# unmeshvrije/scikit-kge

Hardware: AMD Instinct MI355X
Metric: triples/sec (score+grad+update), WN18 TransE d=200, 1/2/4/8 MI355X (higher is better)
Workload: dtype f32; 1 GPU; TransE-L1 d=200 PairwiseStochasticTrainer+AdaGrad, WN18 shape, nb=100 (B=1414), margin 2.0, lr 0.1, device RandomModeSampler(1,[0,1]); step = 1 epoch; global_batch=1414, parallelism=1gpu

## Files before the change

### scikit-kge_amd/csrc/skge_pipe_plan.h

```cpp
#pragma once
#include <stddef.h>
#include <stdint.h>

#include <algorithm>
#include <vector>

#include "../../include/skge_hip.h"
#include "skge_epoch_batches.h"

namespace skge {

constexpr int HOT_REPS = 4, HOT_MIN = 4, HOT_REL = 8, HOT_MAX = 256;

constexpr int SLOT_BUF = 1 << 30;

constexpr int PIPE_WG_GRP = 192;
#ifndef SKGE_PIPE_WG
#define SKGE_PIPE_WG 256
#endif

constexpr int HPIPE_OCC = 2;

struct PipeEnv {
  int fused = -1;
  int rreps = 0;
  bool hole_fft = false;
  bool hole_hot = true;
  size_t lds_fft_wave = 0, lds_fft_wg = 0, lds_direct_wg = 0;
  int shard_words = 0;
};

struct PipeLaunch {
  long long start;
  int count, prev_slots, pprev_slots, nwork, nA, grid;
};

struct PipeBytes {
  size_t ent_rows = 0;
  size_t ent_sum = 0;
  size_t ent_word = 0;
  size_t ent_meta = 0;
  size_t slots = 0;
  size_t rel_rows = 0;
  size_t rel_acc = 0;
  size_t rec = 0, rec_n1 = 0, err = 0, key_copy = 0, stats = 0, viol = 0;
  size_t hot_sum = 0, hot_cnt = 0, hot_val = 0, hot_row = 0;
};

struct PipePlan {
  bool hole = false;
  bool dp = false;
  bool e8 = false;
  bool w32 = false;
  bool grouped = false;
  bool fused = false;
  bool fft = false;
  bool pair = false;
  bool hot = false;
  bool ent_ada = false, rel_ada = false;
  int kq = 1;
  int reps = 1, rw = 0;
  bool rfold = false;
  size_t lds = 0;
  int wpb = 0;
  int hw = 0;
  int N = 0, M = 0, d = 0, nb1 = 0;
  long long T = 0;
  int64_t bs = 0;
  EpochBatches batches;
  std::vector<PipeLaunch> launch;
  PipeBytes bytes;

  int threads() const { return pair ? 128 : (grouped ? PIPE_WG_GRP : SKGE_PIPE_WG); }
  int nlaunch() const { return nb1 + 3; }
  int kernel() const { return hole ? 2 : (fused ? 1 : 0); }

  int score_groups(int n) const {
    if (n <= 0) return 0;
    return pair ? std::max(1, std::min(n, 2 * 16384))
                : std::max(1, std::min((n + wpb - 1) / wpb, 16384));
  }
// ... 26 lines not shown
    const int cprev = b >= 1 ? (int)batches[b - 1].second : 0;
    a.prev_slots = 4 * cprev;
    if (p.fused) {
      const int cpp = b >= 2 ? (int)batches[b - 2].second : 0;
      a.pprev_slots = 4 * cpp;
      a.nwork = a.count + std::max(cprev, cpp);
      a.nA = 0;
      a.grid = std::max(1, (p.M + a.nwork + WPB - 1) / WPB);
      p.launch.push_back(a);
      continue;
    }
    const int a_items = p.M + nhot +
                        (p.hole ? 4 * cprev
                         : p.grouped ? (4 * cprev + 63) / 64 : 4 * cprev);
    auto nBwaves = [&](long long cnt) { return p.pair ? 2 * cnt : (cnt + WPB - 1) / WPB * WPB; };
    const int occ = p.pair ? std::max(4, HPIPE_OCC) : p.fft ? 4 : HPIPE_OCC;
    int a_cap = p.hole && b < nb1 ? std::max(1, (occ * 4 * 256 - (int)nBwaves(batches[b].second)) / WPB - 8) : 16384;
    if (p.hole && b < nb1 && (long long)nBwaves(batches[b].second) > occ * 4 * 256)
      a_cap = std::max(a_cap, 256);
    a.nA = std::max(1, std::min((a_items + WPB - 1) / WPB, std::min(a_cap, 16384)));
    a.grid = a.nA + p.score_groups(a.count);
    p.launch.push_back(a);
  }
}

inline PipePlan pipe_plan(const skge_table_t* ent, const skge_table_t* rel, int d, int64_t T,
                          int nbatches, int flags, bool hole, const PipeEnv& env) {
  PipePlan p;
  p.hole = hole;
  p.dp = (flags & SKGE_PIPE_DP) != 0;
  p.batches = epoch_batches(T, nbatches);
  p.nb1 = p.batches.size();
  p.bs = p.batches.bs;
  p.T = T;
  p.d = d;
  const int64_t bs = p.bs, maxb = p.batches.maxb;
  const int nq = d / 4;
  const int N = p.N = ent->rows, M = p.M = rel->rows;
  p.fft = hole && env.hole_fft;
  p.pair = p.fft && d == 200 && 2 * maxb <= 4 * 4 * 256;
  p.e8 = !hole && ent->acc_mode == SKGE_ACC_I8X4;
  p.w32 = rel->acc_mode == SKGE_ACC_I32X2;
  p.kq = (nq + 63) / 64;
  p.grouped = !hole && 4 * bs > 4 * 4096;
  {
    const bool ok = !hole && !p.grouped && nq <= 64 && (long long)N < SLOT_BUF;
    p.fused = ok && !p.dp && (env.fused >= 0 ? env.fused != 0 : nq <= 16);
  }
  p.hot = !p.fused && !p.e8 && !p.dp && (!hole || (p.pair && env.hole_hot));
  p.hw = ((hole ? d / 2 : nq) + 15) / 16 * 16;
  p.ent_ada = ent->opt == SKGE_ADAGRAD && ent->state != nullptr;
  p.rel_ada = rel->opt == SKGE_ADAGRAD;
  p.reps = 1;
  if (hole)
    while (p.reps < 32 && (long long)p.reps * 2048 < bs) p.reps *= 2;
  if (hole && env.rreps) p.reps = std::max(1, env.rreps);
  if (p.grouped) {
    const long long per_row = bs / std::max(1, M);
    while (p.reps < 16 && (long long)p.reps * 256 < per_row) p.reps *= 2;
  }
  p.rfold = p.reps > 1;
  p.rw = hole ? ((d + 2) / 2 + 15) / 16 * 16 : ((p.w32 ? 2 * nq : nq) + 1 + 15) / 16 * 16;
  p.lds = !hole ? 0 : p.pair ? env.lds_fft_wave : p.fft ? env.lds_fft_wg : env.lds_direct_wg;
  p.wpb = p.pair ? 2 : (p.grouped ? PIPE_WG_GRP : SKGE_PIPE_WG) / 64;

  PipeBytes& b = p.bytes;
  b.ent_rows = (size_t)N * d * 4;
  b.ent_sum = (size_t)N * nq * (hole ? 16 : (p.e8 ? 4 : 8));
  b.ent_word = (size_t)N * 4;
  b.ent_meta = (size_t)N * 16;
  b.slots = (size_t)4 * bs * 4;
  b.rel_rows = (size_t)M * d * 4;
// ... 17 lines not shown
```

### scikit-kge_amd/csrc/skge_pipeline.hip

```cpp
#include <algorithm>
#include <cstdlib>
#include <tuple>
#include <type_traits>
#include <vector>

#include "skge_graph_runner.h"
#include "skge_hole.h"
#include "skge_hole_fft.h"
#include "skge_pipe.h"
#include "skge_sampler.h"
#include "skge_transe_l1.h"

namespace skge {

#ifndef SKGE_HPIPE_HOT
#define SKGE_HPIPE_HOT 1
#endif

#ifndef SKGE_PIPE_WAVES_I8
#define SKGE_PIPE_WAVES_I8 7
#endif
#ifndef SKGE_PIPE_WAVES_I16
#define SKGE_PIPE_WAVES_I16 7
#endif
constexpr int pipe_batch_waves(int kq, bool w32, bool e8, bool grp, bool hot, bool dp) {
  return (kq != 1 || w32 || grp || hot || dp) ? 0 : (e8 ? SKGE_PIPE_WAVES_I8 : SKGE_PIPE_WAVES_I16);
}
template <int KQ, bool W32, bool E8, bool GRP = false, bool HOT = false, bool DP = false>
__global__ __launch_bounds__(GRP ? PIPE_WG_GRP : SKGE_PIPE_WG)
__attribute__((amdgpu_waves_per_eu(pipe_batch_waves(KQ, W32, E8, GRP, HOT, DP),
                                   pipe_batch_waves(KQ, W32, E8, GRP, HOT, DP))))
void k_pipe_batch(PipeArgs a) {
  const int wpb = blockDim.x >> 6;
  const int l = lane_id();
  const int d = a.d, nq = d >> 2;
  const int rcw = W32 ? 2 * nq : nq;
  const int g = launch_id(a), gp = g - 1;
  const int cp = a.b & 1, pp = cp ^ 1;
  const int rd = a.b & 1;
  const int rw = a.b < a.nb1 ? rd ^ 1 : 0;
  const int ra_prev = (g - 1) % 3, ra_cur = g % 3, ra_old = (g - 2) % 3;
  const int nB = (int)gridDim.x - a.nA;
  const int blk = (int)blockIdx.x;
  const int blk_a = blk, blk_b = blk - a.nA;
  if (blk < a.nA) {
    const int nR = a.R.rows;
    const int* const ownp = a.E.own[pp];
    const int nH = a.E.nhot, nRH = nR + nH;
    const int total = nRH + (ownp ? (a.prev_slots + 63) / 64 : a.prev_slots);
    const int wa = blk_a * wpb + (threadIdx.x >> 6);
    const unsigned long long ta0 = a.trace ? now_10ns() : 0ull;
    const bool wt = a.b < a.nb1;
    if (a.b == a.nb1 && wa == 0) {
      fold_shards(a.nviol_shards, a.nviol_total);
      advance_key(a);
    }
    for (int w = wa; w < total; w += a.nA * wpb) {
      if (w < nR) {
        rel_publish<KQ, W32>(a, w, rd, rw, ra_prev, ra_old);
      } else if (w < nRH) {
        if (HOT) apply_hot<KQ>(a.E, w - nR, g, d);
      } else if (ownp) {
        const int i = 64 * (w - nRH) + l;
        const int r = i < a.prev_slots ? a.E.touched[pp][i] : -1;
        const bool mine = r >= 0 && ownp[r] == i;
        uint64_t m = __ballot(mine);
        if (GRP) {
          while (m) {
            const int rank = __popcll(m & ((1ull << l) - 1ull));
            const bool take = ((m >> l) & 1ull) && rank < GRP_ROWS;
            const uint64_t tk = __ballot(take);
            const int n = __popcll(tk);
            int src = 0;
            {
              uint64_t t2 = tk;
              for (int j = 0; j < GRP_ROWS && t2; ++j) {
                const int k = __ffsll((unsigned long long)t2) - 1;
                t2 &= t2 - 1;
                if (l == j) src = k;
              }
            }
            const int rl = __builtin_amdgcn_ds_bpermute(src << 2, r);
            claim_and_apply_rows<KQ, E8>(a.E, pp, rl, n, d, gp, wt);
            m &= ~tk;
          }
        } else {
          while (m) {
            const int k = __ffsll((unsigned long long)m) - 1;
            m &= m - 1;
            const int row = __builtin_amdgcn_readlane(r, k);
            claim_and_apply<KQ, E8>(a.E, pp, row, d, gp, wt);
          }
        }
      } else {
        const int row = __builtin_amdgcn_readfirstlane(a.E.touched[pp][w - nRH]);
        if (row >= 0) claim_and_apply<KQ, E8>(a.E, pp, row, d, gp, wt);
      }
    }
    if (a.trace && l == 0) {
      unsigned long long* tr = a.trace + 2 + 6 * (size_t)a.count + 2 * (size_t)wa;
      tr[0] = ta0;
      tr[1] = now_10ns();
    }
    return;
  }
  int* const cnt_cp = opaque_ptr(a.E.cnt[cp]);
  int* const tch_cp = opaque_ptr(a.E.touched[cp]);
  int* const pend_cp = opaque_ptr(a.E.pend[cp]);
  int* const own_cp = a.E.own[cp];
  unsigned long long* const racc0 = opaque_ptr(a.R.acc[ra_cur]);
  const size_t rrep = (size_t)a.R.rows * a.R.rw;
  const int rmask = a.R.reps - 1;
  unsigned long long* const esum = opaque_ptr(a.E.sum[cp]);
  const __amdgpu_buffer_rsrc_t rec_rs = __builtin_amdgcn_make_buffer_rsrc(
      const_cast<int4*>(a.rec + a.start), 0, a.count * 16, 0x00020000);
  const __amdgpu_buffer_rsrc_t rec1_rs = __builtin_amdgcn_make_buffer_rsrc(
      const_cast<int*>(a.rec_n1 + a.start), 0, a.count * 4, 0x00020000);
  int nv = 0;
  const int lo = DP ? a.lo : 0, hi = DP ? a.hi : a.count;
  for (int w = lo + blk_b * wpb + (threadIdx.x >> 6); w < hi; w += nB * wpb) {
    unsigned long long* const racc = racc0 + (size_t)(w & rmask) * rrep;
    unsigned long long tt[4];
    if (a.trace) tt[0] = now_10ns();
    const u32x4 rx = __builtin_amdgcn_raw_buffer_load_b128(rec_rs, w * 16, 0, 0);
    const int r1 = (int)__builtin_amdgcn_raw_buffer_load_b32(rec1_rs, w * 4, 0, 0);
    const int4 r4 = make_int4((int)rx.x, (int)rx.y, (int)rx.z, (int)rx.w);
    __builtin_amdgcn_sched_barrier(0);
    const int s = __builtin_amdgcn_readfirstlane(r4.x);
    const int o = __builtin_amdgcn_readfirstlane(r4.y);
    const int p = __builtin_amdgcn_readfirstlane(r4.z);
    const int neg0 = __builtin_amdgcn_readfirstlane(r4.w);
    const int neg1 = __builtin_amdgcn_readfirstlane(r1);
    const int n0r = neg0 >= 0 ? neg0 : s, n1r = neg1 >= 0 ? neg1 : o;
    float4 es[KQ], eo[KQ], rp[KQ], fs[KQ], fo[KQ], ra[KQ];
    unsigned long long rsv[KQ], rsw[KQ], rcnt;
    rel_row_issue<KQ, W32>(a.R, p, d, rd, ra_prev, rp, ra, rsv, rsw, rcnt);
    __builtin_amdgcn_sched_barrier(0);
    load_row4_buf<KQ>(a.E.P, s, d, es);
    load_row4_buf<KQ>(a.E.P, o, d, eo);
    load_row4_buf<KQ>(a.E.P, n0r, d, fs);
    load_row4_buf<KQ>(a.E.P, n1r, d, fo);
    const int rr = sel4(l & 3, s, o, n0r, n1r);
    const int mark = a.E.pend[pp][rr];
    const int dn = __hip_atomic_load(a.E.done + rr, __ATOMIC_RELAXED, __HIP_MEMORY_SCOPE_AGENT);
    int hx = -1;
    if (HOT) hx = a.E.hot[rr];
    __builtin_amdgcn_sched_barrier(0);
    {
      int c;
      rel_row_finish<KQ, W32>(a.R, d, rsv, rsw, rcnt, rp, ra, c);
    }
    __builtin_amdgcn_sched_barrier(0);
    const uint64_t pend = __ballot(mark == gp) & 0xfull;
    const uint64_t unpub = pend & ~__ballot(dn == gp);
    if (a.trace) tt[1] = now_10ns();
    if (pend) {
#pragma unroll 1
      for (int k = 0; k < 4; ++k) {
        if (!((unpub >> k) & 1ull)) continue;
        ensure_applied<KQ, E8>(a.E, pp, sel4(k, s, o, n0r, n1r), d, gp, a.err);
      }
      if (pend & 1ull) load_row4_sc1<KQ>(a.E.P, s, d, es);
      if (pend & 2ull) load_row4_sc1<KQ>(a.E.P, o, d, eo);
      if (pend & 4ull) load_row4_sc1<KQ>(a.E.P, n0r, d, fs);
      if (pend & 8ull) load_row4_sc1<KQ>(a.E.P, n1r, d, fo);
    }
    if (HOT) {
      const uint64_t hm = __ballot(hx >= 0) & 0xfull;
#pragma unroll 1
      for (int k = 0; k < 4; ++k) {
        if (!((hm >> k) & 1ull)) continue;
        float4 hv[KQ], ha[KQ];
        hot_value<KQ>(a.E, __builtin_amdgcn_readlane(hx, k), g, d, hv, ha);
#pragma unroll
        for (int m = 0; m < KQ; ++m) {
          if (k == 0) es[m] = hv[m];
          if (k == 1) eo[m] = hv[m];
          if (k == 2) fs[m] = hv[m];
          if (k == 3) fo[m] = hv[m];
        }
      }
    }
    if (a.trace) tt[2] = now_10ns();
    float ps, n0, n1;
    float4 gp4[KQ], g0[KQ], g1[KQ];
    int v0, v1;
    l1_scores_signs<KQ>(es, eo, fs, fo, rp, ps, n0, n1, gp4, g0, g1);
    l1_decide(ps, n0, n1, neg0, neg1, a.margin, v0, v1);
    if (a.trace) tt[3] = now_10ns();
    if (DP && a.dprec) {
      uint32_t* out = a.dprec + (size_t)(w - lo) * pipe_dp_record_words(d);
      if (l == 0) out[0] = (uint32_t)(v0 | (v1 << 1));
      if (v0 + v1 > 0) {
#pragma unroll
        for (int m = 0; m < KQ; ++m) {
          const int q = 64 * m + l;
          if (q < nq) out[1 + q] = tern4q(gp4[m]) | (tern4q(g0[m]) << 8) | (tern4q(g1[m]) << 16);
        }
      }
    }
    {
      const int cE = sel4(l, v0 + 2 * v1, 2 * v0 + v1, v0, v1);
      const int rE = sel4(l, s, o, neg0, neg1);
      if (HOT && l < 4 && hx >= 0) {
        if (cE > 0) atomicAdd(a.E.hcnt[g % 3] + hx * HOT_REPS + (w & (HOT_REPS - 1)), cE);
        tch_cp[4 * w + l] = -1;
      } else if (l < 4) {
        commit_slot(cnt_cp, tch_cp, rE, cE, 4 * w + l);
        if (cE > 0) {
          pend_cp[rE] = g;
          if (own_cp) own_cp[rE] = 4 * w + l;
        }
      } else if (l == 4 && v0 + v1 > 0) {
        atomicAdd(racc + (size_t)p * a.R.rw + rcw, (unsigned long long)(2 * (v0 + v1)));
      }
    }
    if (v0 + v1 > 0) {
      nv += v0 + v1;
      float4 cs[KQ], co[KQ], c0[KQ], c1[KQ], cr[KQ];
      const float fv0 = (float)v0, fv1 = (float)v1;
#pragma unroll
      for (int m = 0; m < KQ; ++m)
        l1_contrib(fv0, fv1, gp4[m], g0[m], g1[m], cs[m], co[m], c0[m], c1[m], cr[m]);
      if (E8) {
        unsigned int* es8 = reinterpret_cast<unsigned int*>(esum);
        acc_row4_i8<KQ>(es8, s, cs, d);
        acc_row4_i8<KQ>(es8, o, co, d);
        if (v0) acc_row4_i8<KQ>(es8, neg0, c0, d);
        if (v1) acc_row4_i8<KQ>(es8, neg1, c1, d);
      } else {
        auto base = [&](int k, int row) {
          const int h = HOT ? __builtin_amdgcn_readlane(hx, k) : -1;
          return h >= 0 ? a.E.hsum[g % 3] + ((size_t)h * HOT_REPS + (w & (HOT_REPS - 1))) * a.E.hw
                        : esum + (size_t)row * nq;
        };
        add_row4_i16<KQ>(base(0, s), cs, d);
        add_row4_i16<KQ>(base(1, o), co, d);
        if (v0) add_row4_i16<KQ>(base(2, neg0), c0, d);
        if (v1) add_row4_i16<KQ>(base(3, neg1), c1, d);
      }
      l1_add_rel<KQ, W32>(racc + (size_t)p * a.R.rw, cr, d);
    }
    if (a.trace) {
      if (l == 0) {
        unsigned long long* tr = a.trace + 2 + 6 * (size_t)w;
        tr[0] = tt[0]; tr[1] = tt[1]; tr[2] = tt[2]; tr[3] = tt[3]; tr[4] = now_10ns();
        tr[5] = pend | ((unsigned long long)(v0 + v1 > 0) << 8);
      }
    }
  }
  if (l == 0 && nv) {
    atomicAdd(shard_of(a.nviol_shards), nv);
    if (a.stats_viol) atomicAdd(shard_of(a.stats_viol), nv);
  }
}


template <int KQ, bool E8>
__device__ __forceinline__ void load_sums_raw(const void* S, int row, int d,
                                              unsigned long long (&sv)[KQ]) {
  const int l = lane_id(), nq = d >> 2;
#pragma unroll
  for (int m = 0; m < KQ; ++m) {
    const int q = 64 * m + l, qc = q < nq ? q : nq - 1;
    if (E8)
      sv[m] = reinterpret_cast<const unsigned int*>(S)[(size_t)row * nq + qc];
    else
      sv[m] = reinterpret_cast<const unsigned long long*>(S)[(size_t)row * nq + qc];
  }
}

template <int KQ, bool E8>
__device__ __forceinline__ void decode_sums(const unsigned long long (&sv)[KQ], int d,
                                            float4 (&sm)[KQ]) {
  const int l = lane_id(), nq = d >> 2;
#pragma unroll
// ... 520 lines not shown
  return SKGE_OK;
}

}

using namespace skge;

struct skge_pipe_runner : GraphRunnerCore {
  PipePlan plan;
  int* err = nullptr;
  int* stats = nullptr;
  const int* trip = nullptr;
  long long T = 0;
  int half = 0, n_ent = 0, ntries = 0;
  uint64_t seed = 0;
  uint64_t* epoch_key = nullptr;
  uint64_t* key_copy = nullptr;
  TripleSet set;
  int kind = SAMPLER_RANDOM;
  Pools pl = {nullptr, nullptr, 0};
  int4* rec = nullptr;
  int* rec_n1 = nullptr;
  std::vector<PipeArgs> batch;
  bool invalid = false;
  int nlaunch() const { return plan.nlaunch(); }
};

template <class F, class... C>
static bool with_flags(F& f, std::tuple<C...>) {
  return f(C{}...);
}
template <class F, class... C, class... B>
static bool with_flags(F& f, std::tuple<C...>, bool b, B... rest) {
  return b ? with_flags(f, std::tuple<C..., std::true_type>{}, rest...)
           : with_flags(f, std::tuple<C..., std::false_type>{}, rest...);
}
template <class F, class... B>
static bool with_kq_flags(F& f, int kq, B... flags) {
  if (kq <= 1) return with_flags(f, std::tuple<std::integral_constant<int, 1>>{}, flags...);
  if (kq <= 2) return with_flags(f, std::tuple<std::integral_constant<int, 2>>{}, flags...);
  return with_flags(f, std::tuple<std::integral_constant<int, 4>>{}, flags...);
}

constexpr bool pipe_fused_exists(int kq) { return kq == 1; }
constexpr bool pipe_batch_exists(bool e8, bool hot, bool dp) {
  return !(e8 && hot) && !(dp && hot);
}

static bool no_instance(const char* kernel, const PipePlan& p, bool hot) {
  set_error("pipelined runner: no %s instance for kq %d, w32 %d, e8 %d, grouped %d, hot %d, dp %d",
            kernel, p.kq, p.w32, p.e8, p.grouped, hot, p.dp);
  return false;
}

static bool launch_fused(const skge_pipe_runner* r, dim3 gr, hipStream_t st, const PipeArgs& a) {
  const dim3 bl(SKGE_PIPE_WG);
  auto go = [&](auto K, auto W32, auto E8) {
    if constexpr (pipe_fused_exists(K())) {
      hipLaunchKernelGGL((k_pipe_fused<K(), W32(), E8()>), gr, bl, 0, st, a);
      return true;
    } else {
      return false;
    }
  };
  const PipePlan& p = r->plan;
  return with_kq_flags(go, p.kq, p.w32, p.e8) || no_instance("k_pipe_fused", p, false);
}

static bool launch_pipe_batch(const skge_pipe_runner* r, dim3 gr, hipStream_t st,
                              const PipeArgs& a) {
  const PipePlan& p = r->plan;
  const dim3 bl(p.threads());
  auto go = [&](auto K, auto W32, auto E8, auto GRP, auto HOT, auto DP) {
    if constexpr (pipe_batch_exists(E8(), HOT(), DP())) {
      hipLaunchKernelGGL((k_pipe_batch<K(), W32(), E8(), GRP(), HOT(), DP()>), gr, bl, 0, st, a);
      return true;
    } else {
      return false;
    }
  };
  const bool hot = a.E.nhot > 0;
  return with_kq_flags(go, p.kq, p.w32, p.e8, p.grouped, hot, p.dp) ||
         no_instance("k_pipe_batch", p, hot);
}

static bool enqueue_epoch(const skge_pipe_runner* r, hipStream_t st, hipEvent_t* ev, int* stats,
                          int trace_launch = -1, unsigned long long* trace = nullptr) {
  const PipePlan& p = r->plan;
  int i = 0;
  if (ev) (void)hipEventRecord(ev[i], st);
  launch_pipe_sample(st, r->trip, r->T, r->half, r->seed, (const uint64_t*)r->epoch_key, r->set,
                     r->kind, r->pl, r->n_ent, r->ntries, r->rec, r->rec_n1, (const int*)r->err,
                     r->key_copy);
  ++i;
  if (ev) (void)hipEventRecord(ev[i], st);
  for (size_t k = 0; k < r->batch.size(); ++k, ++i) {
    PipeArgs a = r->batch[k];
    if (stats) {
      const int sh = NSHARD * SHARD_STRIDE;
      a.E.claims = stats + (3 * i) * sh;
      a.R.updated = stats + (3 * i + 1) * sh;
      a.stats_viol = stats + (3 * i + 2) * sh;
    }
    if (trace && i == trace_launch) a.trace = trace;
    if (ev) a.key_next = nullptr;
    const dim3 gr(p.launch[k].grid);
    if (p.hole) {
      launch_hole_pipe(km_for(a.d), p.pair, p.fft, gr, dim3(p.threads()), p.lds, st, a);
    } else if (!(p.fused ? launch_fused(r, gr, st, a) : launch_pipe_batch(r, gr, st, a))) {
      return false;
    }
    if (p.rfold && a.count > 0) {
      const size_t words = (size_t)a.R.rows * a.R.rw;
      if (p.hole)
        launch_rel_fold_f(dim3((unsigned)std::min<size_t>((2 * words + 255) / 256, 4096)), st, a);
      else
        hipLaunchKernelGGL(k_rel_fold, dim3((unsigned)std::min<size_t>((words + 255) / 256, 4096)),
                           dim3(256), 0, st, a);
    }
    if (ev) (void)hipEventRecord(ev[i + 1], st);
  }
  if (ev) {
    hipLaunchKernelGGL(k_pipe_advance, dim3(1), dim3(1), 0, st, r->epoch_key);
    (void)hipEventRecord(ev[i + 1], st);
  }
  return true;
}

__global__ __launch_bounds__(256) void k_hot_io(PipeTab t, int nb1, const uint64_t* ek, int d,
                                                int back) {
  const int g0 = (int)(*ek * (uint64_t)(nb1 + 1)) + 2;
  const int b = (g0 - 1) & 1;
// ... 136 lines not shown
    h[rows[j]] = j;
  }
  t.hw = r->plan.hw;
  int* dh = (int*)r->alloc(sz.ent_word, true);
  int* dr = (int*)r->alloc(nh * sz.hot_row, true);
  for (int k = 0; k < 3; ++k) {
    t.hsum[k] = (unsigned long long*)r->alloc(nh * sz.hot_sum, true);
    t.hcnt[k] = (int*)r->alloc(nh * sz.hot_cnt, true);
  }
  for (int k = 0; k < 2; ++k) {
    t.hP[k] = (float*)r->alloc(nh * sz.hot_val, true);
    t.hA[k] = r->plan.ent_ada ? (float*)r->alloc(nh * sz.hot_val, true) : nullptr;
  }
  if (!r->alloc_ok ||
      hipMemcpy(dh, h.data(), (size_t)N * 4, hipMemcpyHostToDevice) != hipSuccess ||
      hipMemcpy(dr, rows.data(), (size_t)nh * 4, hipMemcpyHostToDevice) != hipSuccess)
    return false;
  t.hot = dh;
  t.hot_rows = dr;
  t.nhot = nh;
  return true;
}

static PipeEnv pipe_env(int d, bool hole) {
  PipeEnv e;
  if (const char* f = getenv("SKGE_PIPE_FUSED")) e.fused = atoi(f) != 0;
  if (const char* q = getenv("SKGE_HPIPE_RREPS")) e.rreps = atoi(q);
  e.hole_hot = SKGE_HPIPE_HOT != 0;
  e.shard_words = NSHARD * SHARD_STRIDE;
  if (hole) {
    e.hole_fft = hole_use_fft(d);
    e.lds_fft_wave = hole_fft_lds_bytes(d, 1);
    e.lds_fft_wg = hole_fft_lds_bytes(d, SKGE_PIPE_WG / 64);
    e.lds_direct_wg = (size_t)(SKGE_PIPE_WG / 64) * hole_pos_lds_floats(d) * sizeof(float);
  }
  return e;
}

static bool pipe_check_tables(const skge_table_t* ent, const skge_table_t* rel, int d, int flags,
                              bool hole, int af, int kind) {
  if (flags & ~SKGE_PIPE_DP) return set_error("pipelined runner: unknown flags %d", flags), false;
  const bool dp = (flags & SKGE_PIPE_DP) != 0;
  if (dp && hole)
    return set_error("pipelined runner: the data-parallel form is TransE-L1 only"), false;
  if (dp && kind != SKGE_SAMPLER_RANDOM)
    return set_error("pipelined runner: the data-parallel form (SKGE_PIPE_DP) draws RANDOM negatives "
                "only, not sampler kind %d", kind), false;
  if (!ent || !rel) return set_error("pipelined runner: NULL table"), false;
// ... 112 lines not shown
  q.A[0] = p.rel_ada ? rel->state : nullptr;
  a.rec = r->rec;
  a.rec_n1 = r->rec_n1;
  a.nb1 = p.nb1;
  a.epoch_key = p.dp ? r->epoch_key : r->key_copy;
  a.d = p.d;
  a.margin = margin;
  a.nviol_total = nviol_total;
  a.err = r->err;
  a.af = af;
  a.pair_r1 = 1;
  for (int b = 0; b <= p.nb1; ++b) {
    const PipeLaunch& L = p.launch[b];
    a.b = b;
    a.start = L.start;
    a.count = L.count;
    a.lo = 0;
    a.hi = a.count;
    a.key_next = !p.dp && b == p.nb1 ? r->epoch_key : nullptr;
    a.prev_slots = L.prev_slots;
    a.pprev_slots = L.pprev_slots;
    a.nwork = L.nwork;
    a.nA = L.nA;
    r->batch.push_back(a);
  }
}

static skge_pipe_runner_t* pipe_create(void* stream, const skge_table_t* ent,
                                       const skge_table_t* rel, int d, const int* trip, int64_t T,
                                       const void* set, int64_t set_capacity, int nbatches,
                                       uint64_t seed, uint64_t* epoch_key, float margin,
                                       int ntries, int* nviol_total, int flags, bool hole, int af,
                                       const skge_sampler_t* smp = nullptr) {
  if (check_sampler(smp, "pipelined runner")) return nullptr;
  const int kind = smp ? smp->kind : SKGE_SAMPLER_RANDOM;
  if (!pipe_check_tables(ent, rel, d, flags, hole, af, kind)) return nullptr;
  if (!check_runner_args("pipelined runner", trip, set, epoch_key, T, INT64_MAX, nbatches,
                         set_capacity, 4, ntries, stream))
    return nullptr;
  if (!pipe_check_batch(ent, T, nbatches)) return nullptr;
  hipStream_t st = as_stream(stream);
  std::unique_ptr<skge_pipe_runner> r(new skge_pipe_runner());
  r->plan = pipe_plan(ent, rel, d, T, nbatches, flags, hole, pipe_env(d, hole));
  const PipePlan& p = r->plan;
  r->kind = kind;
  if (kind != SKGE_SAMPLER_RANDOM)
    r->pl = {(const long long*)smp->pool_off, smp->pool_ent, smp->n_rel};
  r->trip = trip;
  r->T = T;
  r->half = perm_half(T);
  r->n_ent = p.N;
  r->ntries = ntries;
  r->seed = seed;
  r->epoch_key = epoch_key;
  r->set = triple_set_view(set, set_capacity);
  PipeArgs a = {};
  if (!pipe_alloc(r.get(), st, a, trip, smp))
    return fail("pipelined runner: device allocation failed");
  if (r->alloc_bytes != p.total(a.E.nhot))
    return fail("pipelined runner: plan and allocations disagree (%zu bytes planned for %d hot "
                "rows, %zu requested)", p.total(a.E.nhot), a.E.nhot, r->alloc_bytes);
  if (a.E.nhot > 0) pipe_plan_launches(r->plan, a.E.nhot);
  a.tw = p.fft ? hole_fft_table(d) : nullptr;
  if (p.fft && !a.tw) return fail("pipelined runner: HolE FFT twiddle table allocation failed");
  pipe_fill_args(r.get(), a, ent, rel, margin, nviol_total, af);
  if (p.dp) {
// ... 91 lines not shown
                                                       const int* trip, int64_t T, const void* set,
                                                       int64_t set_capacity, int nbatches,
                                                       uint64_t seed, uint64_t* epoch_key,
                                                       float margin, int ntries,
                                                       int* nviol_total) {
  return skge_pipe_runner_create_ex(stream, ent, rel, d, trip, T, set, set_capacity, nbatches,
                                    seed, epoch_key, margin, ntries, nviol_total, 0);
}

static int refuse_invalid(const skge_pipe_runner* r) {
  set_error("pipelined runner: an earlier epoch failed (error word set or launch failed); the "
            "tables hold that epoch's partial updates and the runner refuses further runs -- "
            "restore the parameters and build a new runner");
  (void)r;
  return SKGE_EINVAL;
}

extern "C" int skge_pipe_runner_run(skge_pipe_runner_t* r, void* stream, int nepochs) {
  SKGE_CHECK_ARG(r && (r->exec || r->plan.dp), "bad runner");
  SKGE_CHECK_ARG(!r->plan.dp, "data-parallel runner: drive it with skge_pipe_runner_dp_*");
  if (r->invalid) return refuse_invalid(r);
  hipStream_t st = as_stream(stream);
  hot_io(r, st, false);
  const hipError_t e = r->launch(st, nepochs);
  hot_io(r, st, true);
  fused_finalize(r, st);
  if (e != hipSuccess) {
    r->invalid = true;
    set_error("pipelined runner: hipGraphLaunch failed: %s (runner now invalid)",
              hipGetErrorString(e));
    return SKGE_EHIP;
  }
  SKGE_CHECK_LAUNCH("pipelined runner finalize");
  return SKGE_OK;
}

extern "C" int skge_pipe_runner_profile(skge_pipe_runner_t* r, void* stream, float* us_out,
                                        int* stats_out, int n, int trace_launch,
                                        uint64_t* trace_out, int64_t trace_len) {
  SKGE_CHECK_ARG(r && us_out && stats_out, "NULL argument");
  SKGE_CHECK_ARG(!r->plan.dp, "profile(): not for the data-parallel form");
  if (r->invalid) return refuse_invalid(r);
  const int nl = r->nlaunch();
  SKGE_CHECK_ARG(n >= nl, "output arrays need nlaunches entries");
  hipStream_t st = as_stream(stream);
  std::vector<hipEvent_t> ev(nl + 1, nullptr);
// ... 163 lines not shown
```

Before: 217.6 million triples/s.

## Fold next-epoch negative sampling into pipelined batch kernels as extra workgroups

Moves the per-epoch negative-sample draw out of its standalone kernel and into extra workgroups appended to the last batch launches (and the final publish launch), drawing records for the next epoch while the current one finishes. The first epoch's draw is enqueued once before the graph launch. The batch kernel body is split into a shared include so a tail variant can run both the batch work and the sampling. This removes a serialized launch and its idle gap per epoch, at the cost of added workgroups competing with scoring work and more complex key and error handling across epochs.

```diff
diff --git a/scikit-kge_amd/csrc/skge_pipe_batch_body.h b/scikit-kge_amd/csrc/skge_pipe_batch_body.h
--- /dev/null
+++ b/scikit-kge_amd/csrc/skge_pipe_batch_body.h
@@ -0,0 +1,223 @@
+  const int wpb = blockDim.x >> 6;
+  const int l = lane_id();
+  const int d = a.d, nq = d >> 2;
+  const int rcw = W32 ? 2 * nq : nq;
+  const int g = launch_id(a), gp = g - 1;
+  const int cp = a.b & 1, pp = cp ^ 1;
+  const int rd = a.b & 1;
+  const int rw = a.b < a.nb1 ? rd ^ 1 : 0;
+  const int ra_prev = (g - 1) % 3, ra_cur = g % 3, ra_old = (g - 2) % 3;
+  const int nB = (TAIL ? tail_nwg : (int)gridDim.x) - a.nA;
+  const int blk = (int)blockIdx.x;
+  const int blk_a = blk, blk_b = blk - a.nA;
+  if (blk < a.nA) {
+    const int nR = a.R.rows;
+    const int* const ownp = a.E.own[pp];
+    const int nH = a.E.nhot, nRH = nR + nH;
+    const int total = nRH + (ownp ? (a.prev_slots + 63) / 64 : a.prev_slots);
+    const int wa = blk_a * wpb + (threadIdx.x >> 6);
+    const unsigned long long ta0 = a.trace ? now_10ns() : 0ull;
+    const bool wt = a.b < a.nb1;
+    if (a.b == a.nb1 && wa == 0) {
+      fold_shards(a.nviol_shards, a.nviol_total);
+      advance_key(a);
+    }
+    for (int w = wa; w < total; w += a.nA * wpb) {
+      if (w < nR) {
+        rel_publish<KQ, W32>(a, w, rd, rw, ra_prev, ra_old);
+      } else if (w < nRH) {
+        if (HOT) apply_hot<KQ>(a.E, w - nR, g, d);
+      } else if (ownp) {
+        const int i = 64 * (w - nRH) + l;
+        const int r = i < a.prev_slots ? a.E.touched[pp][i] : -1;
+        const bool mine = r >= 0 && ownp[r] == i;
+        uint64_t m = __ballot(mine);
+        if (GRP) {
+          while (m) {
+            const int rank = __popcll(m & ((1ull << l) - 1ull));
+            const bool take = ((m >> l) & 1ull) && rank < GRP_ROWS;
+            const uint64_t tk = __ballot(take);
+            const int n = __popcll(tk);
+            int src = 0;
+            {
+              uint64_t t2 = tk;
+              for (int j = 0; j < GRP_ROWS && t2; ++j) {
+                const int k = __ffsll((unsigned long long)t2) - 1;
+                t2 &= t2 - 1;
+                if (l == j) src = k;
+              }
+            }
+            const int rl = __builtin_amdgcn_ds_bpermute(src << 2, r);
+            claim_and_apply_rows<KQ, E8>(a.E, pp, rl, n, d, gp, wt);
+            m &= ~tk;
+          }
+        } else {
+          while (m) {
+            const int k = __ffsll((unsigned long long)m) - 1;
+            m &= m - 1;
+            const int row = __builtin_amdgcn_readlane(r, k);
+            claim_and_apply<KQ, E8>(a.E, pp, row, d, gp, wt);
+          }
+        }
+      } else {
+        const int row = __builtin_amdgcn_readfirstlane(a.E.touched[pp][w - nRH]);
+        if (row >= 0) claim_and_apply<KQ, E8>(a.E, pp, row, d, gp, wt);
+      }
+    }
+    if (a.trace && l == 0) {
+      unsigned long long* tr = a.trace + 2 + 6 * (size_t)a.count + 2 * (size_t)wa;
+      tr[0] = ta0;
+      tr[1] = now_10ns();
+    }
+    return;
+  }
+  int* const cnt_cp = opaque_ptr(a.E.cnt[cp]);
+  int* const tch_cp = opaque_ptr(a.E.touched[cp]);
+  int* const pend_cp = opaque_ptr(a.E.pend[cp]);
+  int* const own_cp = a.E.own[cp];
+  unsigned long long* const racc0 = opaque_ptr(a.R.acc[ra_cur]);
+  const size_t rrep = (size_t)a.R.rows * a.R.rw;
+  const int rmask = a.R.reps - 1;
+  unsigned long long* const esum = opaque_ptr(a.E.sum[cp]);
+  const __amdgpu_buffer_rsrc_t rec_rs = __builtin_amdgcn_make_buffer_rsrc(
+      const_cast<int4*>(a.rec + a.start), 0, a.count * 16, 0x00020000);
+  const __amdgpu_buffer_rsrc_t rec1_rs = __builtin_amdgcn_make_buffer_rsrc(
+      const_cast<int*>(a.rec_n1 + a.start), 0, a.count * 4, 0x00020000);
+  int nv = 0;
+  const int lo = DP ? a.lo : 0, hi = DP ? a.hi : a.count;
+  for (int w = lo + blk_b * wpb + (threadIdx.x >> 6); w < hi; w += nB * wpb) {
+    unsigned long long* const racc = racc0 + (size_t)(w & rmask) * rrep;
+    unsigned long long tt[4];
+    if (a.trace) tt[0] = now_10ns();
+    const u32x4 rx = __builtin_amdgcn_raw_buffer_load_b128(rec_rs, w * 16, 0, 0);
+    const int r1 = (int)__builtin_amdgcn_raw_buffer_load_b32(rec1_rs, w * 4, 0, 0);
+    const int4 r4 = make_int4((int)rx.x, (int)rx.y, (int)rx.z, (int)rx.w);
+    __builtin_amdgcn_sched_barrier(0);
+    const int s = __builtin_amdgcn_readfirstlane(r4.x);
+    const int o = __builtin_amdgcn_readfirstlane(r4.y);
+    const int p = __builtin_amdgcn_readfirstlane(r4.z);
+    int neg0 = __builtin_amdgcn_readfirstlane(r4.w);
+    int neg1 = __builtin_amdgcn_readfirstlane(r1);
+    if (TAIL && tail_stop) neg0 = neg1 = -1;
+    const int n0r = neg0 >= 0 ? neg0 : s, n1r = neg1 >= 0 ? neg1 : o;
+    float4 es[KQ], eo[KQ], rp[KQ], fs[KQ], fo[KQ], ra[KQ];
+    unsigned long long rsv[KQ], rsw[KQ], rcnt;
+    rel_row_issue<KQ, W32>(a.R, p, d, rd, ra_prev, rp, ra, rsv, rsw, rcnt);
+    __builtin_amdgcn_sched_barrier(0);
+    load_row4_buf<KQ>(a.E.P, s, d, es);
+    load_row4_buf<KQ>(a.E.P, o, d, eo);
+    load_row4_buf<KQ>(a.E.P, n0r, d, fs);
+    load_row4_buf<KQ>(a.E.P, n1r, d, fo);
+    const int rr = sel4(l & 3, s, o, n0r, n1r);
+    const int mark = a.E.pend[pp][rr];
+    const int dn = __hip_atomic_load(a.E.done + rr, __ATOMIC_RELAXED, __HIP_MEMORY_SCOPE_AGENT);
+    int hx = -1;
+    if (HOT) hx = a.E.hot[rr];
+    __builtin_amdgcn_sched_barrier(0);
+    {
+      int c;
+      rel_row_finish<KQ, W32>(a.R, d, rsv, rsw, rcnt, rp, ra, c);
+    }
+    __builtin_amdgcn_sched_barrier(0);
+    const uint64_t pend = __ballot(mark == gp) & 0xfull;
+    const uint64_t unpub = pend & ~__ballot(dn == gp);
+    if (a.trace) tt[1] = now_10ns();
+    if (pend) {
+#pragma unroll 1
+      for (int k = 0; k < 4; ++k) {
+        if (!((unpub >> k) & 1ull)) continue;
+        ensure_applied<KQ, E8>(a.E, pp, sel4(k, s, o, n0r, n1r), d, gp, a.err);
+      }
+      if (pend & 1ull) load_row4_sc1<KQ>(a.E.P, s, d, es);
+      if (pend & 2ull) load_row4_sc1<KQ>(a.E.P, o, d, eo);
+      if (pend & 4ull) load_row4_sc1<KQ>(a.E.P, n0r, d, fs);
+      if (pend & 8ull) load_row4_sc1<KQ>(a.E.P, n1r, d, fo);
+    }
+    if (HOT) {
+      const uint64_t hm = __ballot(hx >= 0) & 0xfull;
+#pragma unroll 1
+      for (int k = 0; k < 4; ++k) {
+        if (!((hm >> k) & 1ull)) continue;
+        float4 hv[KQ], ha[KQ];
+        hot_value<KQ>(a.E, __builtin_amdgcn_readlane(hx, k), g, d, hv, ha);
+#pragma unroll
+        for (int m = 0; m < KQ; ++m) {
+          if (k == 0) es[m] = hv[m];
+          if (k == 1) eo[m] = hv[m];
+          if (k == 2) fs[m] = hv[m];
+          if (k == 3) fo[m] = hv[m];
+        }
+      }
+    }
+    if (a.trace) tt[2] = now_10ns();
+    float ps, n0, n1;
+    float4 gp4[KQ], g0[KQ], g1[KQ];
+    int v0, v1;
+    l1_scores_signs<KQ>(es, eo, fs, fo, rp, ps, n0, n1, gp4, g0, g1);
+    l1_decide(ps, n0, n1, neg0, neg1, a.margin, v0, v1);
+    if (a.trace) tt[3] = now_10ns();
+    if (DP && a.dprec) {
+      uint32_t* out = a.dprec + (size_t)(w - lo) * pipe_dp_record_words(d);
+      if (l == 0) out[0] = (uint32_t)(v0 | (v1 << 1));
+      if (v0 + v1 > 0) {
+#pragma unroll
+        for (int m = 0; m < KQ; ++m) {
+          const int q = 64 * m + l;
+          if (q < nq) out[1 + q] = tern4q(gp4[m]) | (tern4q(g0[m]) << 8) | (tern4q(g1[m]) << 16);
+        }
+      }
+    }
+    {
+      const int cE = sel4(l, v0 + 2 * v1, 2 * v0 + v1, v0, v1);
+      const int rE = sel4(l, s, o, neg0, neg1);
+      if (HOT && l < 4 && hx >= 0) {
+        if (cE > 0) atomicAdd(a.E.hcnt[g % 3] + hx * HOT_REPS + (w & (HOT_REPS - 1)), cE);
+        tch_cp[4 * w + l] = -1;
+      } else if (l < 4) {
+        commit_slot(cnt_cp, tch_cp, rE, cE, 4 * w + l);
+        if (cE > 0) {
+          pend_cp[rE] = g;
+          if (own_cp) own_cp[rE] = 4 * w + l;
+        }
+      } else if (l == 4 && v0 + v1 > 0) {
+        atomicAdd(racc + (size_t)p * a.R.rw + rcw, (unsigned long long)(2 * (v0 + v1)));
+      }
+    }
+    if (v0 + v1 > 0) {
+      nv += v0 + v1;
+      float4 cs[KQ], co[KQ], c0[KQ], c1[KQ], cr[KQ];
+      const float fv0 = (float)v0, fv1 = (float)v1;
+#pragma unroll
+      for (int m = 0; m < KQ; ++m)
+        l1_contrib(fv0, fv1, gp4[m], g0[m], g1[m], cs[m], co[m], c0[m], c1[m], cr[m]);
+      if (E8) {
+        unsigned int* es8 = reinterpret_cast<unsigned int*>(esum);
+        acc_row4_i8<KQ>(es8, s, cs, d);
+        acc_row4_i8<KQ>(es8, o, co, d);
+        if (v0) acc_row4_i8<KQ>(es8, neg0, c0, d);
+        if (v1) acc_row4_i8<KQ>(es8, neg1, c1, d);
+      } else {
+        auto base = [&](int k, int row) {
+          const int h = HOT ? __builtin_amdgcn_readlane(hx, k) : -1;
+          return h >= 0 ? a.E.hsum[g % 3] + ((size_t)h * HOT_REPS + (w & (HOT_REPS - 1))) * a.E.hw
+                        : esum + (size_t)row * nq;
+        };
+        add_row4_i16<KQ>(base(0, s), cs, d);
+        add_row4_i16<KQ>(base(1, o), co, d);
+        if (v0) add_row4_i16<KQ>(base(2, neg0), c0, d);
+        if (v1) add_row4_i16<KQ>(base(3, neg1), c1, d);
+      }
+      l1_add_rel<KQ, W32>(racc + (size_t)p * a.R.rw, cr, d);
+    }
+    if (a.trace) {
+      if (l == 0) {
+        unsigned long long* tr = a.trace + 2 + 6 * (size_t)w;
+        tr[0] = tt[0]; tr[1] = tt[1]; tr[2] = tt[2]; tr[3] = tt[3]; tr[4] = now_10ns();
+        tr[5] = pend | ((unsigned long long)(v0 + v1 > 0) << 8);
+      }
+    }
+  }
+  if (l == 0 && nv) {
+    atomicAdd(shard_of(a.nviol_shards), nv);
+    if (a.stats_viol) atomicAdd(shard_of(a.stats_viol), nv);
+  }
diff --git a/scikit-kge_amd/csrc/skge_pipe_plan.h b/scikit-kge_amd/csrc/skge_pipe_plan.h
--- a/scikit-kge_amd/csrc/skge_pipe_plan.h
+++ b/scikit-kge_amd/csrc/skge_pipe_plan.h
@@ -18,6 +18,13 @@
 #ifndef SKGE_PIPE_WG
 #define SKGE_PIPE_WG 256
 #endif
+
+constexpr int PIPE_RESIDENT_WAVES = 256 * 4 * 7;
+#ifndef SKGE_PIPE_DRAW_SHARE
+#define SKGE_PIPE_DRAW_SHARE 0
+#endif
+constexpr int DRAW_TAIL_SHARE = SKGE_PIPE_DRAW_SHARE;
+constexpr int PIPE_FIX_WGS = 8;
 
 constexpr int HPIPE_OCC = 2;
 
@@ -28,11 +35,17 @@
   bool hole_hot = true;
   size_t lds_fft_wave = 0, lds_fft_wg = 0, lds_direct_wg = 0;
   int shard_words = 0;
+  bool random_draw = true;
+  int draw_share = -1;
+  bool ahead = true;
 };
 
 struct PipeLaunch {
   long long start;
   int count, prev_slots, pprev_slots, nwork, nA, grid;
+  long long draw_lo, draw_hi;
+  int nX;
+  bool tail;
 };
 
 struct PipeBytes {
@@ -57,6 +70,8 @@
   bool fft = false;
   bool pair = false;
   bool hot = false;
+  bool ahead = false;
+  int draw_share = DRAW_TAIL_SHARE;
   bool ent_ada = false, rel_ada = false;
   int kq = 1;
   int reps = 1, rw = 0;
@@ -129,6 +144,23 @@
     a.grid = a.nA + p.score_groups(a.count);
     p.launch.push_back(a);
   }
+  if (!p.ahead) return;
+  const int lb = nb1 - 1;
+  const long long start_last = p.launch[lb].start;
+  const bool small = 4ll * p.launch[lb].count <= PIPE_RESIDENT_WAVES;
+  auto draws = [&](PipeLaunch& a, long long lo, long long hi) {
+    a.draw_lo = lo;
+    a.draw_hi = hi;
+    if (hi > lo) a.nX = (int)std::min<long long>((hi - lo + p.threads() - 1) / p.threads(), 8192);
+  };
+  const long long n_tail = small ? std::min(start_last, p.T * p.draw_share / 100) : 0;
+  draws(p.launch[lb], 0, n_tail);
+  draws(p.launch[nb1], n_tail, p.T);
+  p.launch[0].nX = std::max(p.launch[0].nX, PIPE_FIX_WGS);
+  for (PipeLaunch& a : p.launch) {
+    a.tail = a.nX > 0;
+    a.grid += a.nX;
+  }
 }
 
 inline PipePlan pipe_plan(const skge_table_t* ent, const skge_table_t* rel, int d, int64_t T,
@@ -155,6 +187,8 @@
     p.fused = ok && !p.dp && (env.fused >= 0 ? env.fused != 0 : nq <= 16);
   }
   p.hot = !p.fused && !p.e8 && !p.dp && (!hole || (p.pair && env.hole_hot));
+  p.ahead = !hole && !p.fused && !p.dp && env.random_draw && env.ahead;
+  if (env.draw_share >= 0) p.draw_share = std::min(env.draw_share, 100);
   p.hw = ((hole ? d / 2 : nq) + 15) / 16 * 16;
   p.ent_ada = ent->opt == SKGE_ADAGRAD && ent->state != nullptr;
   p.rel_ada = rel->opt == SKGE_ADAGRAD;
diff --git a/scikit-kge_amd/csrc/skge_pipeline.hip b/scikit-kge_amd/csrc/skge_pipeline.hip
--- a/scikit-kge_amd/csrc/skge_pipeline.hip
+++ b/scikit-kge_amd/csrc/skge_pipeline.hip
@@ -26,232 +26,59 @@
 constexpr int pipe_batch_waves(int kq, bool w32, bool e8, bool grp, bool hot, bool dp) {
   return (kq != 1 || w32 || grp || hot || dp) ? 0 : (e8 ? SKGE_PIPE_WAVES_I8 : SKGE_PIPE_WAVES_I16);
 }
+
 template <int KQ, bool W32, bool E8, bool GRP = false, bool HOT = false, bool DP = false>
 __global__ __launch_bounds__(GRP ? PIPE_WG_GRP : SKGE_PIPE_WG)
 __attribute__((amdgpu_waves_per_eu(pipe_batch_waves(KQ, W32, E8, GRP, HOT, DP),
                                    pipe_batch_waves(KQ, W32, E8, GRP, HOT, DP))))
 void k_pipe_batch(PipeArgs a) {
-  const int wpb = blockDim.x >> 6;
-  const int l = lane_id();
-  const int d = a.d, nq = d >> 2;
-  const int rcw = W32 ? 2 * nq : nq;
-  const int g = launch_id(a), gp = g - 1;
-  const int cp = a.b & 1, pp = cp ^ 1;
-  const int rd = a.b & 1;
-  const int rw = a.b < a.nb1 ? rd ^ 1 : 0;
-  const int ra_prev = (g - 1) % 3, ra_cur = g % 3, ra_old = (g - 2) % 3;
-  const int nB = (int)gridDim.x - a.nA;
-  const int blk = (int)blockIdx.x;
-  const int blk_a = blk, blk_b = blk - a.nA;
-  if (blk < a.nA) {
-    const int nR = a.R.rows;
-    const int* const ownp = a.E.own[pp];
-    const int nH = a.E.nhot, nRH = nR + nH;
-    const int total = nRH + (ownp ? (a.prev_slots + 63) / 64 : a.prev_slots);
-    const int wa = blk_a * wpb + (threadIdx.x >> 6);
-    const unsigned long long ta0 = a.trace ? now_10ns() : 0ull;
-    const bool wt = a.b < a.nb1;
-    if (a.b == a.nb1 && wa == 0) {
-      fold_shards(a.nviol_shards, a.nviol_total);
-      advance_key(a);
-    }
-    for (int w = wa; w < total; w += a.nA * wpb) {
-      if (w < nR) {
-        rel_publish<KQ, W32>(a, w, rd, rw, ra_prev, ra_old);
-      } else if (w < nRH) {
-        if (HOT) apply_hot<KQ>(a.E, w - nR, g, d);
-      } else if (ownp) {
-        const int i = 64 * (w - nRH) + l;
-        const int r = i < a.prev_slots ? a.E.touched[pp][i] : -1;
-        const bool mine = r >= 0 && ownp[r] == i;
-        uint64_t m = __ballot(mine);
-        if (GRP) {
-          while (m) {
-            const int rank = __popcll(m & ((1ull << l) - 1ull));
-            const bool take = ((m >> l) & 1ull) && rank < GRP_ROWS;
-            const uint64_t tk = __ballot(take);
-            const int n = __popcll(tk);
-            int src = 0;
-            {
-              uint64_t t2 = tk;
-              for (int j = 0; j < GRP_ROWS && t2; ++j) {
-                const int k = __ffsll((unsigned long long)t2) - 1;
-                t2 &= t2 - 1;
-                if (l == j) src = k;
-              }
-            }
-            const int rl = __builtin_amdgcn_ds_bpermute(src << 2, r);
-            claim_and_apply_rows<KQ, E8>(a.E, pp, rl, n, d, gp, wt);
-            m &= ~tk;
-          }
-        } else {
-          while (m) {
-            const int k = __ffsll((unsigned long long)m) - 1;
-            m &= m - 1;
-            const int row = __builtin_amdgcn_readlane(r, k);
-            claim_and_apply<KQ, E8>(a.E, pp, row, d, gp, wt);
-          }
-        }
-      } else {
-        const int row = __builtin_amdgcn_readfirstlane(a.E.touched[pp][w - nRH]);
-        if (row >= 0) claim_and_apply<KQ, E8>(a.E, pp, row, d, gp, wt);
-      }
-    }
-    if (a.trace && l == 0) {
-      unsigned long long* tr = a.trace + 2 + 6 * (size_t)a.count + 2 * (size_t)wa;
-      tr[0] = ta0;
-      tr[1] = now_10ns();
-    }
+  constexpr bool TAIL = false;
+  constexpr int tail_nwg = 0;
+  constexpr bool tail_stop = false;
+#include "skge_pipe_batch_body.h"
+}
+
+struct TailArgs {
+  uint64_t* key_pub;
+  int4* rec;
+  int* rec_n1;
+  long long T;
+  long long draw_lo, draw_hi;
+  const int* trip;
+  int half, n_ent, ntries;
+  uint64_t seed;
+  TripleSet set;
+  int nX;
+};
+
+template <int KQ, bool W32, bool E8, bool GRP, bool HOT>
+__global__ __launch_bounds__(GRP ? PIPE_WG_GRP : SKGE_PIPE_WG)
+void k_pipe_tail(PipeArgs a, TailArgs t) {
+  constexpr bool TAIL = true, DP = false;
+  const int first_x = (int)gridDim.x - t.nX;
+  const int err = __hip_atomic_load(a.err, __ATOMIC_RELAXED, __HIP_MEMORY_SCOPE_AGENT);
+  if ((int)blockIdx.x < first_x) {
+    if (t.key_pub && blockIdx.x == 0 && threadIdx.x == 0) *t.key_pub = *a.epoch_key;
+    const int tail_nwg = first_x;
+    const bool tail_stop = a.b == 0 && err != 0;
+#include "skge_pipe_batch_body.h"
     return;
   }
-  int* const cnt_cp = opaque_ptr(a.E.cnt[cp]);
-  int* const tch_cp = opaque_ptr(a.E.touched[cp]);
-  int* const pend_cp = opaque_ptr(a.E.pend[cp]);
-  int* const own_cp = a.E.own[cp];
-  unsigned long long* const racc0 = opaque_ptr(a.R.acc[ra_cur]);
-  const size_t rrep = (size_t)a.R.rows * a.R.rw;
-  const int rmask = a.R.reps - 1;
-  unsigned long long* const esum = opaque_ptr(a.E.sum[cp]);
-  const __amdgpu_buffer_rsrc_t rec_rs = __builtin_amdgcn_make_buffer_rsrc(
-      const_cast<int4*>(a.rec + a.start), 0, a.count * 16, 0x00020000);
-  const __amdgpu_buffer_rsrc_t rec1_rs = __builtin_amdgcn_make_buffer_rsrc(
-      const_cast<int*>(a.rec_n1 + a.start), 0, a.count * 4, 0x00020000);
-  int nv = 0;
-  const int lo = DP ? a.lo : 0, hi = DP ? a.hi : a.count;
-  for (int w = lo + blk_b * wpb + (threadIdx.x >> 6); w < hi; w += nB * wpb) {
-    unsigned long long* const racc = racc0 + (size_t)(w & rmask) * rrep;
-    unsigned long long tt[4];
-    if (a.trace) tt[0] = now_10ns();
-    const u32x4 rx = __builtin_amdgcn_raw_buffer_load_b128(rec_rs, w * 16, 0, 0);
-    const int r1 = (int)__builtin_amdgcn_raw_buffer_load_b32(rec1_rs, w * 4, 0, 0);
-    const int4 r4 = make_int4((int)rx.x, (int)rx.y, (int)rx.z, (int)rx.w);
-    __builtin_amdgcn_sched_barrier(0);
-    const int s = __builtin_amdgcn_readfirstlane(r4.x);
-    const int o = __builtin_amdgcn_readfirstlane(r4.y);
-    const int p = __builtin_amdgcn_readfirstlane(r4.z);
-    const int neg0 = __builtin_amdgcn_readfirstlane(r4.w);
-    const int neg1 = __builtin_amdgcn_readfirstlane(r1);
-    const int n0r = neg0 >= 0 ? neg0 : s, n1r = neg1 >= 0 ? neg1 : o;
-    float4 es[KQ], eo[KQ], rp[KQ], fs[KQ], fo[KQ], ra[KQ];
-    unsigned long long rsv[KQ], rsw[KQ], rcnt;
-    rel_row_issue<KQ, W32>(a.R, p, d, rd, ra_prev, rp, ra, rsv, rsw, rcnt);
-    __builtin_amdgcn_sched_barrier(0);
-    load_row4_buf<KQ>(a.E.P, s, d, es);
-    load_row4_buf<KQ>(a.E.P, o, d, eo);
-    load_row4_buf<KQ>(a.E.P, n0r, d, fs);
-    load_row4_buf<KQ>(a.E.P, n1r, d, fo);
-    const int rr = sel4(l & 3, s, o, n0r, n1r);
-    const int mark = a.E.pend[pp][rr];
-    const int dn = __hip_atomic_load(a.E.done + rr, __ATOMIC_RELAXED, __HIP_MEMORY_SCOPE_AGENT);
-    int hx = -1;
-    if (HOT) hx = a.E.hot[rr];
-    __builtin_amdgcn_sched_barrier(0);
-    {
-      int c;
-      rel_row_finish<KQ, W32>(a.R, d, rsv, rsw, rcnt, rp, ra, c);
-    }
-    __builtin_amdgcn_sched_barrier(0);
-    const uint64_t pend = __ballot(mark == gp) & 0xfull;
-    const uint64_t unpub = pend & ~__ballot(dn == gp);
-    if (a.trace) tt[1] = now_10ns();
-    if (pend) {
-#pragma unroll 1
-      for (int k = 0; k < 4; ++k) {
-        if (!((unpub >> k) & 1ull)) continue;
-        ensure_applied<KQ, E8>(a.E, pp, sel4(k, s, o, n0r, n1r), d, gp, a.err);
-      }
-      if (pend & 1ull) load_row4_sc1<KQ>(a.E.P, s, d, es);
-      if (pend & 2ull) load_row4_sc1<KQ>(a.E.P, o, d, eo);
-      if (pend & 4ull) load_row4_sc1<KQ>(a.E.P, n0r, d, fs);
-      if (pend & 8ull) load_row4_sc1<KQ>(a.E.P, n1r, d, fo);
-    }
-    if (HOT) {
-      const uint64_t hm = __ballot(hx >= 0) & 0xfull;
-#pragma unroll 1
-      for (int k = 0; k < 4; ++k) {
-        if (!((hm >> k) & 1ull)) continue;
-        float4 hv[KQ], ha[KQ];
-        hot_value<KQ>(a.E, __builtin_amdgcn_readlane(hx, k), g, d, hv, ha);
-#pragma unroll
-        for (int m = 0; m < KQ; ++m) {
-          if (k == 0) es[m] = hv[m];
-          if (k == 1) eo[m] = hv[m];
-          if (k == 2) fs[m] = hv[m];
-          if (k == 3) fo[m] = hv[m];
-        }
-      }
-    }
-    if (a.trace) tt[2] = now_10ns();
-    float ps, n0, n1;
-    float4 gp4[KQ], g0[KQ], g1[KQ];
-    int v0, v1;
-    l1_scores_signs<KQ>(es, eo, fs, fo, rp, ps, n0, n1, gp4, g0, g1);
-    l1_decide(ps, n0, n1, neg0, neg1, a.margin, v0, v1);
-    if (a.trace) tt[3] = now_10ns();
-    if (DP && a.dprec) {
-      uint32_t* out = a.dprec + (size_t)(w - lo) * pipe_dp_record_words(d);
-      if (l == 0) out[0] = (uint32_t)(v0 | (v1 << 1));
-      if (v0 + v1 > 0) {
-#pragma unroll
-        for (int m = 0; m < KQ; ++m) {
-          const int q = 64 * m + l;
-          if (q < nq) out[1 + q] = tern4q(gp4[m]) | (tern4q(g0[m]) << 8) | (tern4q(g1[m]) << 16);
-        }
-      }
-    }
-    {
-      const int cE = sel4(l, v0 + 2 * v1, 2 * v0 + v1, v0, v1);
-      const int rE = sel4(l, s, o, neg0, neg1);
-      if (HOT && l < 4 && hx >= 0) {
-        if (cE > 0) atomicAdd(a.E.hcnt[g % 3] + hx * HOT_REPS + (w & (HOT_REPS - 1)), cE);
-        tch_cp[4 * w + l] = -1;
-      } else if (l < 4) {
-        commit_slot(cnt_cp, tch_cp, rE, cE, 4 * w + l);
-        if (cE > 0) {
-          pend_cp[rE] = g;
-          if (own_cp) own_cp[rE] = 4 * w + l;
-        }
-      } else if (l == 4 && v0 + v1 > 0) {
-        atomicAdd(racc + (size_t)p * a.R.rw + rcw, (unsigned long long)(2 * (v0 + v1)));
-      }
-    }
-    if (v0 + v1 > 0) {
-      nv += v0 + v1;
-      float4 cs[KQ], co[KQ], c0[KQ], c1[KQ], cr[KQ];
-      const float fv0 = (float)v0, fv1 = (float)v1;
-#pragma unroll
-      for (int m = 0; m < KQ; ++m)
-        l1_contrib(fv0, fv1, gp4[m], g0[m], g1[m], cs[m], co[m], c0[m], c1[m], cr[m]);
-      if (E8) {
-        unsigned int* es8 = reinterpret_cast<unsigned int*>(esum);
-        acc_row4_i8<KQ>(es8, s, cs, d);
-        acc_row4_i8<KQ>(es8, o, co, d);
-        if (v0) acc_row4_i8<KQ>(es8, neg0, c0, d);
-        if (v1) acc_row4_i8<KQ>(es8, neg1, c1, d);
-      } else {
-        auto base = [&](int k, int row) {
-          const int h = HOT ? __builtin_amdgcn_readlane(hx, k) : -1;
-          return h >= 0 ? a.E.hsum[g % 3] + ((size_t)h * HOT_REPS + (w & (HOT_REPS - 1))) * a.E.hw
-                        : esum + (size_t)row * nq;
-        };
-        add_row4_i16<KQ>(base(0, s), cs, d);
-        add_row4_i16<KQ>(base(1, o), co, d);
-        if (v0) add_row4_i16<KQ>(base(2, neg0), c0, d);
-        if (v1) add_row4_i16<KQ>(base(3, neg1), c1, d);
-      }
-      l1_add_rel<KQ, W32>(racc + (size_t)p * a.R.rw, cr, d);
-    }
-    if (a.trace) {
-      if (l == 0) {
-        unsigned long long* tr = a.trace + 2 + 6 * (size_t)w;
-        tr[0] = tt[0]; tr[1] = tt[1]; tr[2] = tt[2]; tr[3] = tt[3]; tr[4] = now_10ns();
-        tr[5] = pend | ((unsigned long long)(v0 + v1 > 0) << 8);
-      }
-    }
-  }
-  if (l == 0 && nv) {
-    atomicAdd(shard_of(a.nviol_shards), nv);
-    if (a.stats_viol) atomicAdd(shard_of(a.stats_viol), nv);
+  const long long tid = (long long)((int)blockIdx.x - first_x) * blockDim.x + threadIdx.x;
+  const long long nth = (long long)t.nX * blockDim.x;
+  if (a.b == 0 && err) {
+    for (long long j = a.count + tid; j < t.T; j += nth) {
+      t.rec[j].w = -1;
+      t.rec_n1[j] = -1;
+    }
+  }
+  if (t.draw_lo < t.draw_hi) {
+    const uint64_t ek = *a.epoch_key + 1;
+    const int ntries = err ? 0 : t.ntries;
+    const Perm pm = {(uint64_t)t.T, t.half, epoch_perm_key(t.seed, ek)};
+    const uint64_t skey = epoch_sample_key(t.seed, ek);
+    for (long long j = t.draw_lo + tid; j < t.draw_hi; j += nth)
+      sample_record(t.trip, pm, skey, t.set, t.n_ent, ntries, j, t.rec, t.rec_n1);
   }
 }
 
@@ -818,6 +645,7 @@
   int4* rec = nullptr;
   int* rec_n1 = nullptr;
   std::vector<PipeArgs> batch;
+  std::vector<TailArgs> tail;
   bool invalid = false;
   int nlaunch() const { return plan.nlaunch(); }
 };
@@ -864,11 +692,17 @@
 }
 
 static bool launch_pipe_batch(const skge_pipe_runner* r, dim3 gr, hipStream_t st,
-                              const PipeArgs& a) {
+                              const PipeArgs& a, const TailArgs* t = nullptr) {
   const PipePlan& p = r->plan;
   const dim3 bl(p.threads());
   auto go = [&](auto K, auto W32, auto E8, auto GRP, auto HOT, auto DP) {
     if constexpr (pipe_batch_exists(E8(), HOT(), DP())) {
+      if constexpr (!DP()) {
+        if (t) {
+          hipLaunchKernelGGL((k_pipe_tail<K(), W32(), E8(), GRP(), HOT()>), gr, bl, 0, st, a, *t);
+          return true;
+        }
+      }
       hipLaunchKernelGGL((k_pipe_batch<K(), W32(), E8(), GRP(), HOT(), DP()>), gr, bl, 0, st, a);
       return true;
     } else {
@@ -878,6 +712,12 @@
   const bool hot = a.E.nhot > 0;
   return with_kq_flags(go, p.kq, p.w32, p.e8, p.grouped, hot, p.dp) ||
          no_instance("k_pipe_batch", p, hot);
+}
+
+static void enqueue_draw(const skge_pipe_runner* r, hipStream_t st) {
+  launch_pipe_sample(st, r->trip, r->T, r->half, r->seed, (const uint64_t*)r->epoch_key, r->set,
+                     r->kind, r->pl, r->n_ent, r->ntries, r->rec, r->rec_n1, (const int*)r->err,
+                     r->key_copy);
 }
 
 static bool enqueue_epoch(const skge_pipe_runner* r, hipStream_t st, hipEvent_t* ev, int* stats,
@@ -885,9 +725,7 @@
   const PipePlan& p = r->plan;
   int i = 0;
   if (ev) (void)hipEventRecord(ev[i], st);
-  launch_pipe_sample(st, r->trip, r->T, r->half, r->seed, (const uint64_t*)r->epoch_key, r->set,
-                     r->kind, r->pl, r->n_ent, r->ntries, r->rec, r->rec_n1, (const int*)r->err,
-                     r->key_copy);
+  if (ev || !p.ahead) enqueue_draw(r, st);
   ++i;
   if (ev) (void)hipEventRecord(ev[i], st);
   for (size_t k = 0; k < r->batch.size(); ++k, ++i) {
@@ -903,7 +741,8 @@
     const dim3 gr(p.launch[k].grid);
     if (p.hole) {
       launch_hole_pipe(km_for(a.d), p.pair, p.fft, gr, dim3(p.threads()), p.lds, st, a);
-    } else if (!(p.fused ? launch_fused(r, gr, st, a) : launch_pipe_batch(r, gr, st, a))) {
+    } else if (!(p.fused ? launch_fused(r, gr, st, a)
+                         : launch_pipe_batch(r, gr, st, a, p.launch[k].tail ? &r->tail[k] : nullptr))) {
       return false;
     }
     if (p.rfold && a.count > 0) {
@@ -1086,8 +925,11 @@
   return true;
 }
 
-static PipeEnv pipe_env(int d, bool hole) {
+static PipeEnv pipe_env(int d, bool hole, int kind = SKGE_SAMPLER_RANDOM) {
   PipeEnv e;
+  e.random_draw = kind == SKGE_SAMPLER_RANDOM;
+  if (const char* s = getenv("SKGE_PIPE_DRAW_SHARE")) e.draw_share = std::max(0, atoi(s));
+  if (const char* s = getenv("SKGE_PIPE_AHEAD")) e.ahead = atoi(s) != 0;
   if (const char* f = getenv("SKGE_PIPE_FUSED")) e.fused = atoi(f) != 0;
   if (const char* q = getenv("SKGE_HPIPE_RREPS")) e.rreps = atoi(q);
   e.hole_hot = SKGE_HPIPE_HOT != 0;
@@ -1246,7 +1088,25 @@
     a.pprev_slots = L.pprev_slots;
     a.nwork = L.nwork;
     a.nA = L.nA;
+    if (p.ahead && b == 0) a.epoch_key = r->epoch_key;
     r->batch.push_back(a);
+    TailArgs t = {};
+    if (L.tail) {
+      t.key_pub = b == 0 ? r->key_copy : nullptr;
+      t.rec = r->rec;
+      t.rec_n1 = r->rec_n1;
+      t.T = r->T;
+      t.draw_lo = L.draw_lo;
+      t.draw_hi = L.draw_hi;
+      t.trip = r->trip;
+      t.half = r->half;
+      t.n_ent = r->n_ent;
+      t.ntries = r->ntries;
+      t.seed = r->seed;
+      t.set = r->set;
+      t.nX = L.nX;
+    }
+    r->tail.push_back(t);
   }
 }
 
@@ -1265,7 +1125,7 @@
   if (!pipe_check_batch(ent, T, nbatches)) return nullptr;
   hipStream_t st = as_stream(stream);
   std::unique_ptr<skge_pipe_runner> r(new skge_pipe_runner());
-  r->plan = pipe_plan(ent, rel, d, T, nbatches, flags, hole, pipe_env(d, hole));
+  r->plan = pipe_plan(ent, rel, d, T, nbatches, flags, hole, pipe_env(d, hole, kind));
   const PipePlan& p = r->plan;
   r->kind = kind;
   if (kind != SKGE_SAMPLER_RANDOM)
@@ -1403,6 +1263,7 @@
   if (r->invalid) return refuse_invalid(r);
   hipStream_t st = as_stream(stream);
   hot_io(r, st, false);
+  if (r->plan.ahead && nepochs > 0) enqueue_draw(r, st);
   const hipError_t e = r->launch(st, nepochs);
   hot_io(r, st, true);
   fused_finalize(r, st);
```

After: 218.4 million triples/s (median of 6 runs). Within noise of the previous version (+0.4%).
